# kamerkaya/SUPerman

Hardware: AMD Instinct MI355X
Metric: Gray-code subset-steps/sec (dense n=40, d=0.5) at 1/2/4/8 MI355X; rel-err vs CPU (higher is better)
Workload: dtype f64; 1 GPU; dense Ryser/Gray-code exact permanent (-p4/-p6 path), n=40 d=0.50 (double/40_0.50_0), 2^39 Gray steps per step; n=40, kernel_request=dense, preprocessing=0, jit=1, walk=segmented (pattern-specialised), parallelism=dp1: contiguous wave-chunk shards + one RCCL all-reduce

## Files before the change

### superman_amd/csrc/engine.hpp

```cpp
#pragma once
#include <stdint.h>
#include <cstdio>
#include <memory>
#include <mutex>
#include <functional>
#include <string>
#include <vector>

#include "../../include/superman.h"
#include "kernels.hpp"

namespace sup {

void set_error(const std::string& msg);
const char* last_error();
bool env_on(const char* name, bool dflt);

int to_double(const void* mat, sup_dtype t, int n, std::vector<double>& out);

void nw_start(const double* A, int n, double* x0, double* p0);

constexpr int kMaxCachedBits = 4;

enum SegCensus {
// ... 8 lines not shown
  kCenSharedCopy,
  kCenSharedForm,
  kCenHiAdd,
  kCenHiCopy,
  kCenHiForm,
  kCenStart,
  kSegCensusN
};

struct Layout {
  int L;
  int m;
  int h;
  bool fixed = false;
  int cc_cap = kMaxCachedBits;
  uint64_t chunks() const { return 1ull << h; }
};
Layout default_layout(int n);
Layout layout_with_walk(int n, int walk_log2);

struct ProdTree {
  std::vector<int> item_row;
  std::vector<uint32_t> item_sig;
  int tail_lo = 0, tail_hi = 0;
  std::vector<int> a, b;
  std::vector<uint32_t> sig;
  std::vector<uint8_t> item_live, node_live;
  int items() const { return (int)item_row.size(); }
  int K() const { return (int)a.size(); }
  int root() const { return K() ? items() + K() - 1 : (items() ? 0 : -1); }
// ... 28 lines not shown
  int seg_hi = 0;
  double seg_census[kSegCensusN] = {};
  double seg_skip = 0.0;
  int seg_regs = 0;
  int seg_budget = 0;
  std::vector<int> jofs;
  std::vector<double> jtab;
  size_t seg_cbase = 0;
  bool start_tab_on = false;
  std::vector<double> start_tab;
  int seg_kp = 4;
  std::string jit_src;
  uint64_t jit_key = 0;
  uint64_t uid = 0;
  std::vector<int> seg_order;
  bool seg_loop_scratch = false;
};

struct SegChoice {
  std::vector<int> order;
  int b = 0;
  int budget = 0;
  int cc_cap = kMaxCachedBits;
  int hi = 0;
};

int make_plan(const double* A, int n, WalkKind kind, bool identity_map, const Layout& lay, Plan& P,
              const SegChoice* choice = nullptr);

std::vector<int> greedy_walk_order(const double* A, int n, int count);
bool skip_walk_order(const double* A, int n, const Layout& lay, std::vector<int>& out,
                     const std::vector<int>* baseline, double factor);
int improve_sparse_plan(const double* A, int n, const Layout& lay, Plan& P);
int plan_threads();

std::vector<int> seg_walk_order(const double* A, int n, int m, int count, int* b_out, int cc_cap = kMaxCachedBits);
double seg_skip_estimate(const double* A, int n, const std::vector<int>& order, int m, int samples);
double seg_skip_fraction_plan(const Plan& P, int samples);
std::vector<int> seg_row_order(const double* A, int n, const std::vector<int>& walk);
int build_seg(Plan& P, int fixed_budget = 0, int fixed_hi = 0);
bool seg_choice_load(uint64_t key, int* m, SegChoice* c);
bool seg_choice_exists(uint64_t key);
double seg_cold_model(int n);
double seg_cold_predict(int n);
void seg_cost_store(int n, double seconds);
double seg_cost_ratio_load();
void seg_choice_store(uint64_t key, int m, const SegChoice& c);
int auto_decision_load(uint64_t key);
int auto_decision_store(uint64_t key, int seg);
uint64_t jit_toolchain_hash();
int seg_static_bits(int m);
double seg_cx(const Plan& P, int r, uint32_t S);
double seg_cy(const Plan& P, int r, uint32_t S);
double seg_walk_cost(const Plan& P);
int jit_occupancy(int dev, const Plan& P, int* blocks_per_cu, double* compile_ms);
// ... 313 lines not shown
```

### superman_amd/csrc/jit.cpp

```cpp
#include <dlfcn.h>
#include <hip/hiprtc.h>
#include <sched.h>
#include <spawn.h>
#include <sys/stat.h>
#include <sys/wait.h>
#include <unistd.h>

#include <cerrno>

#include <algorithm>
#include <cstring>
#include <fstream>
#include <iterator>
#include <atomic>
#include <chrono>
#include <cmath>
#include <cstdio>
#include <cstdlib>
#include <map>
#include <queue>
#include <memory>
#include <condition_variable>
#include <mutex>
#include <sstream>
// ... 84 lines not shown
  int regs = 0;
  ProdTree outer, inner;
};

inline uint64_t freq(uint32_t s, int b, int cc) {
  uint64_t v = 0;
  for (int c = cc; c <= b && c < 9; ++c)
    if ((s >> c) & 1u) v += c < b ? (1ull << (b - 1 - c)) : 1ull;
  return v;
}

constexpr int kRegs3 = 90;
static const int kRegsMax = std::getenv("SUP_JIT_REGMAX") ? std::atoi(std::getenv("SUP_JIT_REGMAX")) : 170;
constexpr double kOcc2Penalty = 1.02;

SegFit seg_fit(const SegRows& R, int cc, int budget, int budget_hi = -1, SegFit* fit_hi = nullptr) {
  SegFit f;
  f.cc = cc;
  const ClassWeights W(R.b, cc);
  std::vector<int> orow, irow;
  for (int r = R.len0; r < R.r_end; ++r) orow.push_back(r);
  for (int r = 0; r < R.s_end; ++r) irow.push_back(r);
  f.outer = make_tree(orow, R.rsig, R.r_end, R.n, W);
  f.inner = make_tree(irow, R.rsig, R.s_end, R.len0, W);
  struct Val {
    int parent = -1;
    int kids[2] = {-1, -1};
    double fr = 0;
    int cop = 1;
    double own = 0;
    int store = 0;
    bool live = true, fixed = false;
    double F = 0;
  };
// ... 52 lines not shown
      rg += cD;
    }
    *regs = rg;
    return ops;
  };
  for (auto& v : V)
    if (v.live && !v.fixed && v.parent >= 0 && V[v.parent].fr * V[v.parent].cop == v.fr * v.cop) v.live = false;
  for (const int rt : {bx + f.inner.root(), by + f.inner.root()})
    if (f.inner.root() >= 0)
      for (int k : V[rt].kids)
        if (k >= 0 && V[k].live && !V[k].fixed && fD * cD == V[k].fr * V[k].cop) V[k].live = false;
  int regs = 0;
  double ops = total(&regs);
  auto out = [&](SegFit& g, double ops_now, int regs_now) {
    g.cc = cc;
    g.outer = f.outer, g.inner = f.inner;
    auto put = [&](ProdTree& t, int base, int bit) {
      t.item_live.assign(t.items(), 0);
      t.node_live.assign(t.K(), 0);
      for (int j = 0; j < t.items(); ++j)
        if (V[base + j].live && !V[base + j].fixed) t.item_live[j] |= (uint8_t)(1u << bit);
      for (int i = 0; i < t.K(); ++i)
        if (V[base + t.items() + i].live) t.node_live[i] |= (uint8_t)(1u << bit);
    };
    put(g.outer, bo, 0);
    put(g.inner, bx, 0);
    for (int j = 0; j < g.inner.items(); ++j)
      if (V[by + j].live && !V[by + j].fixed) g.inner.item_live[j] |= 2u;
    for (int i = 0; i < g.inner.K(); ++i)
      if (V[by + g.inner.items() + i].live) g.inner.node_live[i] |= 2u;
    g.ops = (ops_now / (double)(1u << R.b) + 1.0) / 2.0;
    g.regs = regs_now;
  };
  bool took_hi = fit_hi == nullptr;
  auto nearest_live = [&](int i) {
    int a = V[i].parent;
    while (a >= 0 && !V[a].live) a = V[a].parent;
    return a;
  };
  auto delta = [&](int i) {
    const int a = nearest_live(i);
    const double fa = a >= 0 ? V[a].fr : fD, ca = a >= 0 ? V[a].cop : cD;
    return V[i].F * (fa * ca / V[i].cop - V[i].fr);
  };
  typedef std::tuple<double, int, int> Entry;
  std::priority_queue<Entry, std::vector<Entry>, std::greater<Entry>> heap;
  std::vector<int> ver(V.size(), 0);
  std::vector<double> dlt(V.size(), 0.0);
  auto push = [&](int i) {
    if (!V[i].live || V[i].fixed) return;
    dlt[i] = delta(i);
    heap.push(Entry{dlt[i] / V[i].store, i, ++ver[i]});
  };
  for (int i = 0; i < (int)V.size(); ++i) push(i);
  std::vector<int> stack;
  for (;;) {
    while (!heap.empty() && std::get<2>(heap.top()) != ver[std::get<1>(heap.top())]) heap.pop();
    const int best = heap.empty() ? -1 : std::get<1>(heap.top());
    const double bd = best < 0 ? 0.0 : dlt[best];
    if (!took_hi && (best < 0 || (bd > 1e-9 && regs <= budget_hi))) out(*fit_hi, ops, regs), took_hi = true;
    if (best < 0 || (bd > 1e-9 && regs <= budget)) break;
    heap.pop();
    V[best].live = false;
    ++ver[best];
    ops += bd, regs -= V[best].store;
    for (int p = V[best].parent; p >= 0; p = V[p].parent) {
      V[p].F += (double)V[p].cop / V[best].cop * V[best].F;
      if (V[p].live) {
        push(p);
        break;
      }
    }
    stack.assign(1, best);
    while (!stack.empty()) {
      const int u = stack.back();
      stack.pop_back();
// ... 8 lines not shown
  out(f, ops, regs);
  return f;
}

std::atomic<long> g_fit_calls{0};
int search_budget() {
  static const int b = std::getenv("SUP_JIT_SEARCH_BUDGET") ? std::atoi(std::getenv("SUP_JIT_SEARCH_BUDGET")) : kRegsMax;
  return b;
}

int max_cached() {
  const char* e = std::getenv("SUP_JIT_MAXCC");
  return e ? std::max(0, std::min(kMaxCachedBits, std::atoi(e))) : kMaxCachedBits;
}

SegFit seg_best(const SegRows& R, int cc_max, int regs_max = kRegsMax) {
  ++g_fit_calls;
  SegFit best;
  double bscore = 1e300;
  for (int cc = 0; cc <= std::min(cc_max, std::max(0, R.b - 1)); ++cc) {
    SegFit hi;
    SegFit lo = seg_fit(R, cc, kRegs3, regs_max, &hi);
    for (SegFit* f : {&lo, &hi}) {
      if (f->regs > regs_max && cc > 0) continue;
      const double score = f->ops * (f->regs <= kRegs3 ? 1.0 : kOcc2Penalty) * (f->regs > regs_max ? 2.0 : 1.0);
      if (score < bscore) bscore = score, best = std::move(*f);
    }
  }
  return best;
}

SegRows seg_rows_of(const double* A, int n, const std::vector<int>& walk, int b) {
  SegRows R;
  R.n = n, R.m = (int)walk.size();
  const std::vector<int> order = seg_row_order(A, n, walk);
  auto nz = [&](int row, int c) { return A[(size_t)row * n + c] != 0.0; };
  R.touched.assign(R.m, {});
  std::vector<char> any1(n, 0);
  for (int k = 0; k < R.m; ++k)
// ... 49 lines not shown
  std::atomic<size_t> next{0};
  auto worker = [&]() {
    for (size_t i = next++; i < count; i = next++) fn(i);
  };
  std::vector<std::thread> th;
  for (int t = 1; t < std::min({plan_threads(), (int)count, max_threads}); ++t) th.emplace_back(worker);
  worker();
  for (auto& t : th) t.join();
}

int seg_search_starts(int n) {
  if (const char* e = std::getenv("SUP_JIT_STARTS")) return std::max(1, std::atoi(e));
  return std::ldexp(1.0, n - 1) * (2.0 * n + 1.0) / 3.7e13 >= 1.0 ? 32 : 3;
}

std::vector<int> seg_walk_order(const double* A, int n, int m, int count, int* b_out, int cc_cap) {
  cc_cap = std::min(cc_cap, max_cached());
  const int nb = n - 1;
  m = std::min(m, nb);
  count = std::min(std::max(count, m), nb);
  std::vector<int> nnz(n, 0);
  for (int c = 0; c < nb; ++c)
    for (int i = 0; i < n; ++i) nnz[c] += A[(size_t)i * n + c] != 0.0;
  auto extend = [&](std::vector<int> order, int upto) {
    std::vector<char> used(n, 0), placed(n, 0);
    for (int c : order) {
      used[c] = 1;
      for (int i = 0; i < n; ++i) placed[i] |= A[(size_t)i * n + c] != 0.0;
    }
    while ((int)order.size() < upto) {
      int best = -1, bnew = 1 << 30;
      for (int c = 0; c < nb; ++c) {
        if (used[c]) continue;
        int nw = 0;
        for (int i = 0; i < n; ++i) nw += !placed[i] && A[(size_t)i * n + c] != 0.0;
        if (nw < bnew || (nw == bnew && nnz[c] < nnz[best])) best = c, bnew = nw;
      }
      used[best] = 1;
      order.push_back(best);
      for (int i = 0; i < n; ++i) placed[i] |= A[(size_t)i * n + best] != 0.0;
    }
    return order;
  };
  auto cost = [&](const std::vector<int>& o, int b) {
    if (nnz[o[0]] == 0) return 1e300;
    if (m < 3) return 0.0;
    const SegFit f = seg_best(seg_rows_of(A, n, std::vector<int>(o.begin(), o.begin() + m), b), cc_cap,
                              search_budget());
    return seg_block_bytes(f, b) > kMaxBlockBytes ? 1e300 : seg_score(f);
  };
  if (m == 0) {
    if (b_out) *b_out = 0;
    return extend({}, count);
  }
  const std::vector<int> cands = seg_b_candidates(m);
  std::vector<std::vector<int>> bests(cands.size());
  std::vector<std::vector<std::pair<double, std::vector<int>>>> finals(cands.size());
  std::vector<double> bcosts(cands.size(), 1e300);
  std::vector<std::vector<std::pair<double, std::vector<int>>>> starts(cands.size());
  auto rank_starts = [&](size_t ci) {
    const int b = cands[ci];
    for (int f = 0; f < nb; ++f) {
      std::vector<int> o = extend({f}, m);
      starts[ci].push_back({cost(o, b), std::move(o)});
    }
// ... 40 lines not shown
    std::atomic<size_t> next{0};
    auto worker = [&]() {
      for (size_t ti = next++; ti < tasks.size(); ti = next++) descend(ti);
    };
    std::vector<std::thread> th;
    for (int t = 1; t < std::min<int>(plan_threads(), (int)tasks.size()); ++t) th.emplace_back(worker);
    worker();
    for (auto& t : th) t.join();
  }
  for (size_t ci = 0; ci < cands.size(); ++ci) finals[ci].clear();
  for (size_t ti = 0; ti < tasks.size(); ++ti) {
    const size_t ci = tasks[ti].first;
    if (bests[ci].empty() || results[ti].first < bcosts[ci] - 1e-12) bcosts[ci] = results[ti].first, bests[ci] = results[ti].second;
    finals[ci].push_back(results[ti]);
  }
  size_t gi = 0;
  for (size_t ci = 1; ci < cands.size(); ++ci)
    if (bcosts[ci] < bcosts[gi] - 1e-12) gi = ci;
  bool integral = true;
  for (size_t i = 0; i < (size_t)n * n && integral; ++i) integral = A[i] == std::floor(A[i]);
  constexpr int kPolishSamples = 8192;
  constexpr int kPolishEvals = 48;
  const int need_free = std::min(3, std::max(0, nb - count));
  auto balanced = [&](const std::vector<int>& full) {
    std::vector<char> wrow(n, 0), used(n, 0);
    for (int k = 0; k < m; ++k)
      for (int i = 0; i < n; ++i) wrow[i] |= A[(size_t)i * n + full[k]] != 0.0;
    for (int c : full) used[c] = 1;
    int free_cols = 0;
    for (int c = 0; c < nb; ++c) {
      if (used[c]) continue;
      bool f = true;
      for (int i = 0; i < n && f; ++i) f = wrow[i] || A[(size_t)i * n + c] == 0.0;
// ... 26 lines not shown
      double bops = cur_ops;
      for (size_t t = 0; t < trials.size() && (int)t < kPolishEvals; ++t) {
        if (cur_ops * 0.85 * std::get<0>(trials[t]) >= best) break;
        const std::vector<int>& o = std::get<2>(trials[t]);
        if (!balanced(extend(o, count))) continue;
        const double keep = 1.0 - seg_skip_estimate(A, n, extend(o, count), m, kPolishSamples);
        const double ops = std::get<1>(trials[t]) ? cur_ops : cost(std::vector<int>(o.begin(), o.begin() + m), bb);
        if (ops < 1e300 && ops * keep < best - 1e-12) best = ops * keep, bi = (int)t, bops = ops;
      }
      if (bi < 0) break;
      beff = best, cur = std::get<2>(trials[bi]), cur_ops = bops;
    }
    bo = extend(cur, count);
    return beff;
  };
  if (integral && count >= m + std::min(6, nb - m)) {
    double beff = 1e300;
    std::vector<int> bo;
    int bb = cands[gi];
    std::vector<std::tuple<double, int, std::vector<int>>> ranked;
    for (size_t ci = 0; ci < cands.size(); ++ci)
      for (const auto& fc : finals[ci]) {
        if (fc.first >= 1e300) continue;
        const std::vector<int> full = extend(fc.second, count);
        const double eff = balanced(full) ? fc.first * (1.0 - seg_skip_estimate(A, n, full, m, kPolishSamples)) : 1e300;
        if (std::getenv("SUP_JIT_VERBOSE"))
          std::fprintf(stderr, "  candidate b=%d ops=%.4f skip=%.3f eff=%.4f\n", cands[ci], fc.first,
                       1.0 - eff / fc.first, eff);
        ranked.emplace_back(eff, cands[ci], full);
        if (eff < beff - 1e-12) beff = eff, bo = full, bb = cands[ci];
// ... 17 lines not shown
          th.emplace_back([&, i] { effs[i] = polish(std::get<2>(starts[i]), std::get<1>(starts[i]), std::get<0>(starts[i])); });
        for (auto& t : th) t.join();
        if (std::getenv("SUP_JIT_VERBOSE"))
          for (size_t i = 0; i < starts.size(); ++i) {
            const std::vector<int>& o = std::get<2>(starts[i]);
            const double ops = cost(std::vector<int>(o.begin(), o.begin() + m), std::get<1>(starts[i]));
            std::fprintf(stderr, "  polished #%zu b=%d eff=%.4f ops=%.4f eff@16384=%.4f\n", i, std::get<1>(starts[i]),
                         effs[i], ops, ops * (1.0 - seg_skip_estimate(A, n, o, m, 16384)));
          }
        size_t bi = 0;
        for (size_t i = 1; i < starts.size(); ++i)
          if (effs[i] < effs[bi] - 1e-12) bi = i;
        beff = effs[bi], bb = std::get<1>(starts[bi]), bo = std::get<2>(starts[bi]);
        if (std::getenv("SUP_JIT_VERBOSE")) std::fprintf(stderr, "  polished eff=%.4f\n", beff);
      }
      if (b_out) *b_out = bb;
      return bo;
    }
  }
  if (b_out) *b_out = cands[gi];
  return extend(bests[gi], count);
}

double seg_skip_fraction_plan(const Plan& P, int samples) {
  const int n = P.n, L = P.lay.L, m = P.lay.m, nb = n - 1;
  const int tail_lo = P.seg_start.empty() ? n : P.seg_start.back();
  if (tail_lo >= n) return 0.0;
  for (const double v : P.cols)
    if (v != std::floor(v)) return 0.0;
  const int h = nb - L - m;
  int skipped = 0;
  std::vector<double> base(n - tail_lo);
  for (int s = 0; s < samples; ++s) {
    const uint64_t a = h > 0 ? ((uint64_t)s * 0x9E3779B97F4A7C15ull) >> (64 - std::min(h, 63)) : 0;
    const uint64_t g = a ^ (a >> 1);
    for (int r = tail_lo; r < n; ++r) {
// ... 923 lines not shown
  const unsigned hb = (unsigned)(P.lay.L + P.lay.m);
  P.start_tab.assign((size_t)C * NP, 0.0);
  const size_t blocks = (size_t)std::min<uint64_t>(C, 64);
  parallel_tasks(blocks, [&](size_t b) {
    for (uint64_t ga = C * b / blocks; ga < C * (b + 1) / blocks; ++ga) {
      double* x = P.start_tab.data() + (size_t)ga * NP;
      for (int j = 0; j < NP; ++j) x[j] = P.x0[j];
      for (uint64_t h = ga ^ (ga >> 1); h; h &= h - 1) {
        const double* col = P.cols.data() + (size_t)(2u * (hb + (unsigned)__builtin_ctzll(h))) * NP;
        for (int j = 0; j < n; ++j) x[j] += col[j];
      }
    }
  });
}

int build_seg(Plan& P, int fixed_budget, int fixed_hi) {
  const int n = P.n, L = P.lay.L, m = P.lay.m;
  if (m < 3) {
    set_error("segmented walk needs >= 3 walk bits");
    return SUP_EINVAL;
  }
  if (P.cols.empty()) return SUP_EINVAL;
  P.start_tab.clear();
  P.start_tab_on = !std::getenv("SUP_JIT_NO_START_TAB") && P.lay.m <= kStartTabMaxWalkBits &&
                   (double)P.lay.chunks() * P.NP * sizeof(double) <= (double)kStartTabMaxBytes;
  P.touched.assign(m, {});
  P.seg_start.assign(1, 0);
  std::vector<char> seen(n, 0);
  int R = 0;
  for (int k = 0; k < m; ++k) {
    const double* col = P.cols.data() + (size_t)(2 * (L + k)) * P.NP;
    for (int j = 0; j < n; ++j)
// ... 45 lines not shown
    }
  }
  P.dyn_rows.clear();
  {
    std::vector<char> in(n, 0);
    for (int k = P.seg_b + 1; k < m; ++k)
      for (int r : P.touched[k]) in[r] = 1;
    for (int j = 0; j < n; ++j)
      if (in[j]) P.dyn_rows.push_back(j);
  }
  SegRows SR;
  SR.n = n, SR.m = m, SR.touched = P.touched;
  SR.len0 = P.seg_start[1], SR.s_end = P.sub_start.back(), SR.r_end = P.seg_start.back();
  seg_rows_finish(SR, P.seg_b);
  const int cc_cap = std::min(max_cached(), P.lay.cc_cap);
  auto finish = [&SR, &cc_cap, n, L, m](Plan& Q, int budget, int hi) {
    SegFit f;
    if (const char* e = std::getenv("SUP_JIT_CC"))
      f = seg_fit(SR, std::max(0, std::min({std::atoi(e), SR.b - 1, kMaxCachedBits})), budget);
    else f = seg_best(SR, cc_cap, budget);
    if (const char* e = std::getenv("SUP_JIT_STORAGE")) f = seg_fit(SR, f.cc, std::max(0, std::atoi(e)));
    Q.outer_tree = std::move(f.outer);
    Q.inner_tree = std::move(f.inner);
    Q.seg_cc = f.cc;
    Q.seg_model_ops = f.ops;
    Q.seg_regs = f.regs;
    Q.seg_budget = budget;
    Q.jofs.assign(m, 0);
    Q.jtab.clear();
    for (int k = 0; k < m; ++k) {
      const std::vector<int>& t = Q.touched[k];
      const size_t blk = (t.size() + 7) & ~(size_t)7;
      Q.jofs[k] = (int)Q.jtab.size();
      Q.jtab.resize(Q.jtab.size() + 2 * std::max<size_t>(blk, 8), 0.0);
      for (size_t i = 0; i < t.size(); ++i) {
        Q.jtab[Q.jofs[k] + i] = Q.cols[(size_t)(2 * (L + k)) * Q.NP + t[i]];
        Q.jtab[Q.jofs[k] + blk + i] = Q.cols[(size_t)(2 * (L + k) + 1) * Q.NP + t[i]];
      }
    }
    Q.seg_cbase = Q.jtab.size();
    Q.seg_kp = 4;
    if (const char* e = std::getenv("SUP_JIT_KP")) Q.seg_kp = std::max(1, std::atoi(e));
    const int hi_max = std::min(3, m - 1 - Q.seg_b);
    if (const char* e = std::getenv("SUP_JIT_HI")) hi = std::max(0, std::min(3, std::atoi(e)));
    bool neg_zero = false;
    for (int j = 0; j < n; ++j) neg_zero = neg_zero || (Q.x0[j] == 0.0 && std::signbit(Q.x0[j]));
    if (neg_zero) hi = 0;
    auto generate = [&Q](int h, std::string* src) {
      Q.seg_hi = h;
      auto g = std::make_unique<Gen>(Q);
      *src = g->source();
      return g;
    };
    auto total = [](const Gen& g) {
      double ops = 0.0;
      for (int c = 0; c < kCenStart; ++c) ops += g.census[c];
      return ops;
    };
    int taken = hi < 0 ? 0 : std::min(hi, hi_max);
// ... 29 lines not shown
    const int rc = jit_code_scan(P, &s);
    std::fprintf(stderr, "  fixed budget %d: ops %.4f rc %d vgprs %d spills %d scratch %dB (loop %d of %d insts)\n",
                 P.seg_budget, P.seg_ops, rc, s.vgprs, s.vgpr_spills, s.scratch_bytes, s.loop_scratch, s.loop_insts);
  }
  if (!fixed && walk_s < 0.01 && P.seg_cc > 3) {
    CodeScan s;
    P.seg_loop_scratch = jit_code_scan(P, &s) != SUP_OK || s.loop_scratch != 0;
  }
  auto ladder = [&](int hi, Plan& out) -> int {
    std::vector<int> budgets;
    for (int b2 = kRegs3 + 12; b2 <= kRegsMax + 60; b2 += 8) budgets.push_back(b2);
    std::vector<Plan> cand(budgets.size(), P);
    parallel_tasks(budgets.size(), [&](size_t i) { finish(cand[i], budgets[i], hi); });
    std::vector<size_t> idx;
    for (size_t i = 0; i < cand.size(); ++i) {
      bool dup = false;
      for (size_t j : idx) dup = dup || cand[j].jit_key == cand[i].jit_key;
      if (!dup) idx.push_back(i);
    }
    std::vector<CodeScan> scans(cand.size());
    std::vector<int> src(cand.size(), SUP_EHIP);
    std::vector<char> done(cand.size(), 0);
    auto compile_one = [&](size_t i) {
      if (done[i]) return;
      const auto t0 = std::chrono::steady_clock::now();
      const double own = t_compile_ms;
      src[i] = jit_code_scan(cand[i], &scans[i]);
      t_compile_ms = own + std::chrono::duration<double, std::milli>(std::chrono::steady_clock::now() - t0).count();
      done[i] = 1;
    };
    auto clean = [&](size_t i) { return done[i] && src[i] == SUP_OK && scans[i].loop_scratch == 0; };
    size_t pp = 0;
    for (size_t k = 0; k < idx.size(); ++k)
// ... 142 lines not shown
```

### superman_amd/csrc/jit_compile.cpp

```cpp
#include <dlfcn.h>
#include <hip/hip_runtime.h>
#include <hip/hiprtc.h>
#include <sched.h>
#include <signal.h>
#include <spawn.h>
#include <sys/stat.h>
#include <sys/wait.h>
#include <unistd.h>

#include <algorithm>
#include <atomic>
#include <cerrno>
#include <chrono>
#include <condition_variable>
#include <cstdio>
#include <cstdlib>
#include <cstring>
#include <fstream>
#include <map>
#include <memory>
#include <mutex>
#include <sstream>
#include <string>
#include <thread>
// ... 382 lines not shown

uint64_t jit_toolchain_hash() {
  static const uint64_t h = toolchain_hash_impl();
  return h;
}

bool seg_choice_load(uint64_t key, int* m, SegChoice* c) {
  const std::string dir = cache_dir();
  if (dir.empty()) return false;
  std::vector<char> buf;
  if (!read_file(dir + "/plan_" + key_hex(key) + ".txt", buf)) return false;
  buf.push_back('\0');
  std::istringstream in(buf.data());
  std::string tag;
  int ver = 0, cnt = 0;
  if (!(in >> tag >> ver >> *m >> c->b >> c->budget >> c->cc_cap >> c->hi >> cnt) || tag != "supseg" || ver != 4 || cnt < 1 ||
      cnt > 64 || c->hi < 0 || c->hi > 3 || c->cc_cap < 0 || c->cc_cap > kMaxCachedBits)
    return false;
  c->order.resize(cnt);
  for (int& v : c->order)
    if (!(in >> v) || v < 0 || v > 63) return false;
  return true;
}

bool seg_choice_exists(uint64_t key) {
  const std::string dir = cache_dir();
  struct stat sb;
  return !dir.empty() && ::stat((dir + "/plan_" + key_hex(key) + ".txt").c_str(), &sb) == 0;
}

void seg_choice_store(uint64_t key, int m, const SegChoice& c) {
  const std::string dir = cache_dir();
  if (dir.empty() || c.order.empty()) return;
  std::ostringstream o;
  o << "supseg 4 " << m << ' ' << c.b << ' ' << c.budget << ' ' << c.cc_cap << ' ' << c.hi << ' ' << c.order.size();
  for (int v : c.order) o << ' ' << v;
  o << '\n';
  const std::string str = o.str();
  write_file_atomic(dir, "plan_" + key_hex(key) + ".txt", std::vector<char>(str.begin(), str.end()));
}

int auto_decision_load(uint64_t key) {
  const std::string dir = cache_dir();
  if (dir.empty()) return -1;
  std::vector<char> buf;
  if (!read_file(dir + "/auto_" + key_hex(key) + ".txt", buf)) return -1;
  buf.push_back('\0');
  std::istringstream in(buf.data());
  std::string tag;
  int ver = 0, v = -1;
// ... 56 lines not shown
```

### superman_amd/csrc/plan.cpp

```cpp
#include "engine.hpp"

#include <algorithm>
#include <atomic>
#include <chrono>
#include <cmath>
#include <cstdio>
#include <cstdlib>
#include <cstring>
#include <map>
#include <memory>
#include <mutex>
#include <thread>
#include <tuple>

#include <unistd.h>

namespace sup {

static thread_local std::string g_err;
void set_error(const std::string& msg) { g_err = msg; }
const char* last_error() { return g_err.c_str(); }

bool env_on(const char* name, bool dflt) {
  const char* e = std::getenv(name);
// ... 342 lines not shown
      for (int v : o) {
        if (v < 0 || v >= nb || seen[v]) return false;
        seen[v] = 1;
      }
      return true;
    };
    if (given_order) {
      if (!valid_order(choice->order)) {
        set_error("walk column order: not m + L distinct flippable columns");
        return SUP_EINVAL;
      }
      order = choice->order;
    } else if (kind == kWalkSeg && choice && valid_order(choice->order) && choice->b >= 0 && choice->b <= m) {
      order = choice->order;
      segb = choice->b;
    } else {
      order = kind == kWalkSeg ? seg_walk_order(A, n, m, m + L, &segb, lay.cc_cap) : greedy_walk_order(A, n, m + L);
    }
    P.seg_b = segb;
    if (kind == kWalkSeg) P.seg_order.assign(order.begin(), order.begin() + (m + L));
    std::vector<char> used(n, 0);
    for (int k = 0; k < m; ++k) P.colmap[L + k] = order[k], used[order[k]] = 1;
    for (int e = 0; e < L; ++e) P.colmap[e] = order[m + e], used[order[m + e]] = 1;
    int e = L + m;
    std::vector<char> top(n, 0);
    if (kind == kWalkSeg || given_order) {
      std::vector<char> wrow(n, 0);
      for (int k = 0; k < (given_order ? m + L : m); ++k)
        for (int i = 0; i < n; ++i) wrow[i] |= A[(size_t)i * n + order[k]] != 0.0;
      for (int c = 0; c < nb && P.integral; ++c) {
        top[c] = 1;
        for (int i = 0; i < n; ++i)
          if (!wrow[i] && A[(size_t)i * n + c] != 0.0) top[c] = 0;
      }
    }
// ... 48 lines not shown

  P.umask = 0;
  for (int j = 0; j < n; ++j) {
    const int i = P.rowperm[j];
    bool lane_touched = false;
    for (int e = 0; e < L; ++e)
      if (A[(size_t)i * n + P.colmap[e]] != 0.0) lane_touched = true;
    if (!lane_touched) P.umask |= 1ull << j;
    uint64_t rm = 0;
    for (int k = 0; k < m; ++k)
      if (A[(size_t)i * n + P.colmap[L + k]] != 0.0) rm |= 1ull << k;
    P.rowmask[j] = rm;
    if ((kind == kWalkSparse || kind == kWalkDense) && !lane_touched && rm == 0 && !no_chunk_ends())
      P.chunk_ends |= 1ull << j;
  }
  if (kind == kWalkSeg) return build_seg(P, choice ? choice->budget : 0, choice ? choice->hi : 0);
  return SUP_OK;
}

static constexpr double kJitMinSavingSec = 3.0;
static constexpr double kAutoRuns = 4.0;
static constexpr double kJitWarmSavingSec = 0.1;
static constexpr int kJitWarmMinN = 30;

static int plan_for_uncached(const double* A, int n, sup_kernel kernel, const Layout& lay, Plan& P, int jit,
                             int ndev, int dev, double min_saving);
static double auto_min_saving(const double* A, int n, const Layout& lay, int jit);

static constexpr double kSegStartOps = 2048.0;

static constexpr int kSegMinChunkBits = 14;
// ... 19 lines not shown
  const int32_t head[] = {7 , n, lay.L, lay.m, (int32_t)lay.fixed, (int32_t)integral};
  f.bytes(head, sizeof head);
  if (integral) {
    f.bytes(A, nn * sizeof(double));
  } else {
    std::vector<unsigned char> pat((nn + 7) / 8, 0);
    for (size_t i = 0; i < nn; ++i)
      if (A[i] != 0.0) pat[i / 8] |= (unsigned char)(1u << (i % 8));
    f.bytes(pat.data(), pat.size());
  }
  const uint64_t k = knob_hash();
  f.bytes(&k, sizeof k);
  return f.h;
}

static int make_seg_plan(const double* A, int n, const Layout& lay, Plan& P) {
  const uint64_t dkey = seg_disk_key(A, n, lay);
  {
    int m2 = 0;
    SegChoice c;
    if (seg_choice_load(dkey, &m2, &c) && m2 >= 3 && m2 <= lay.m + lay.h && (!lay.fixed || m2 == lay.m)) {
      Layout l2 = lay;
      l2.m = m2;
      l2.h = lay.m + lay.h - m2;
      l2.cc_cap = c.cc_cap;
      if (make_plan(A, n, kWalkSeg, false, l2, P, &c) == SUP_OK) return SUP_OK;
    }
  }
  const auto t_cold = std::chrono::steady_clock::now();
  auto plan = [A, n](const Layout& l, Plan& Q) {
    int r = make_plan(A, n, kWalkSeg, false, l, Q);
    if (r == SUP_OK && Q.seg_loop_scratch && l.cc_cap > 3) {
      Layout l3 = l;
      l3.cc_cap = 3;
      r = make_plan(A, n, kWalkSeg, false, l3, Q);
    }
    return r;
  };
  int rc = plan(lay, P);
  if (rc) return rc;
  if (!lay.fixed) {
    const int mmax = std::min(lay.m + lay.h - kSegMinChunkBits, 31);
    int m2 = lay.m;
    while (m2 < mmax && std::ldexp(P.seg_model_ops, m2) < 32.0 * kSegStartOps) ++m2;
    if (m2 != lay.m) {
      Layout l2 = lay;
      l2.m = m2;
      l2.h = lay.m + lay.h - m2;
      Plan s2;
      if (plan(l2, s2) == SUP_OK) {
        auto eff = [](const Plan& q) {
          return (1.0 - q.seg_skip) * (q.seg_model_ops + std::ldexp(kSegStartOps, -q.lay.m));
        };
        if (eff(s2) < eff(P)) P = std::move(s2);
      }
    }
  }
  SegChoice c;
  c.order = P.seg_order;
  c.b = P.seg_b;
  c.budget = P.seg_budget;
  c.hi = P.seg_hi;
  c.cc_cap = P.lay.cc_cap;
  seg_choice_store(dkey, P.lay.m, c);
  const double cold_s = std::chrono::duration<double>(std::chrono::steady_clock::now() - t_cold).count();
  seg_cost_store(n, cold_s);
  if (std::getenv("SUP_JIT_VERBOSE"))
    std::fprintf(stderr, "cold segmented plan n=%d: %.3f s (compiles %.3f s wall on this thread)\n", n, cold_s,
                 jit_compile_ms_thread() * 1e-3);
  return SUP_OK;
}

namespace {
struct PlanKey {
  uint64_t hash;
  int n, kernel, L, m, jit, ndev;
  bool fixed;
  uint64_t knobs;
  bool operator<(const PlanKey& o) const {
    return std::tie(hash, n, kernel, L, m, jit, ndev, fixed, knobs) <
           std::tie(o.hash, o.n, o.kernel, o.L, o.m, o.jit, o.ndev, o.fixed, o.knobs);
// ... 92 lines not shown
    active = jit == 0 && n >= kJitWarmMinN && walk_s >= kJitWarmSavingSec;
    if (!active) return;
    key = seg_disk_key(A, n, lay) ^ (0x9e3779b97f4a7c15ull * (uint64_t)(1 + (int)kernel)) ^
          ((uint64_t)std::max(ndev, 1) << 48);
    recorded = auto_decision_load(key);
  }
  bool store(bool seg) const {
    if (active && recorded < 0) return auto_decision_store(key, seg ? 1 : 0) == 1;
    return seg;
  }
};

static int plan_for_uncached(const double* A, int n, sup_kernel kernel, const Layout& lay, Plan& P, int jit,
                             int ndev, int dev, double min_saving) {
  std::vector<WalkKind> kinds;
  auto make_seg = [&](Plan& s) { return make_seg_plan(A, n, lay, s); };
  switch (kernel) {
    case SUP_KERNEL_SKIPPER: {
      int rc = make_plan(A, n, kWalkSkip, false, lay, P);
      if (rc) return rc;
      const bool integral = P.integral;
      if (integral && n >= 10 &&
          ops_seconds(gray_steps(n), walk_cost(P), kSkipEfficiency * kLaneOpsPerSec) >= kSkipSearchMinSec) {
        SegChoice c;
        Plan Q;
        if (skip_walk_order(A, n, lay, c.order, nullptr, 0.5) && make_plan(A, n, kWalkSkip, false, lay, Q, &c) == SUP_OK)
          P = std::move(Q);
      }
      if (jit < 0 || n < 10 || lay.m < 3) return SUP_OK;
      const double steps = gray_steps(n, ndev);
      double skip_cost = walk_cost(P) / (integral ? kSkipPriceEfficiency : 1.0);
// ... 105 lines not shown
```

Measured before the change: 2966 billion gray-steps/s.

## Add deep simulated-annealing walk-order search for segmented JIT plans

Adds a deep search mode for the segmented walk order. For large n, or when JIT is requested, it runs parallel simulated-annealing walks over column orders, seeded from the plain search's finalists, and prunes weak b candidates between rounds. The deep order is compiled and checked against the plain order, and the one with the lower modeled effective ops is kept. The aim is fewer per-step operations in the generated kernel, at the cost of much longer cold planning time. It also bumps the cached choice format and adds an ops-only early exit to the fit.

```diff
diff --git a/superman_amd/csrc/engine.hpp b/superman_amd/csrc/engine.hpp
--- a/superman_amd/csrc/engine.hpp
+++ b/superman_amd/csrc/engine.hpp
@@ -46,6 +46,8 @@
   int h;
   bool fixed = false;
   int cc_cap = kMaxCachedBits;
+  bool deep = false;
+  bool order_only = false;
   uint64_t chunks() const { return 1ull << h; }
 };
 Layout default_layout(int n);
@@ -104,6 +106,9 @@
   uint64_t jit_key = 0;
   uint64_t uid = 0;
   std::vector<int> seg_order;
+  int seg_search = 0;
+  std::vector<int> seg_plain_order;
+  int seg_plain_b = 0;
   bool seg_loop_scratch = false;
 };
 
@@ -113,6 +118,8 @@
   int budget = 0;
   int cc_cap = kMaxCachedBits;
   int hi = 0;
+  int search = 0;
+  double must_beat = 1e300;
 };
 
 int make_plan(const double* A, int n, WalkKind kind, bool identity_map, const Layout& lay, Plan& P,
@@ -124,11 +131,20 @@
 int improve_sparse_plan(const double* A, int n, const Layout& lay, Plan& P);
 int plan_threads();
 
-std::vector<int> seg_walk_order(const double* A, int n, int m, int count, int* b_out, int cc_cap = kMaxCachedBits);
+struct SegSearch {
+  bool deep = false;
+  bool deep_ran = false;
+  SegChoice plain;
+  std::vector<SegChoice> per_b;
+};
+std::vector<int> seg_walk_order(const double* A, int n, int m, int count, int* b_out, int cc_cap = kMaxCachedBits,
+                                SegSearch* search = nullptr);
+bool seg_search_deep(int n, bool asked);
+int deep_budget();
 double seg_skip_estimate(const double* A, int n, const std::vector<int>& order, int m, int samples);
 double seg_skip_fraction_plan(const Plan& P, int samples);
 std::vector<int> seg_row_order(const double* A, int n, const std::vector<int>& walk);
-int build_seg(Plan& P, int fixed_budget = 0, int fixed_hi = 0);
+int build_seg(Plan& P, int fixed_budget = 0, int fixed_hi = 0, double must_beat = 1e300);
 bool seg_choice_load(uint64_t key, int* m, SegChoice* c);
 bool seg_choice_exists(uint64_t key);
 double seg_cold_model(int n);
diff --git a/superman_amd/csrc/jit.cpp b/superman_amd/csrc/jit.cpp
--- a/superman_amd/csrc/jit.cpp
+++ b/superman_amd/csrc/jit.cpp
@@ -122,10 +122,17 @@
 static const int kRegsMax = std::getenv("SUP_JIT_REGMAX") ? std::atoi(std::getenv("SUP_JIT_REGMAX")) : 170;
 constexpr double kOcc2Penalty = 1.02;
 
-SegFit seg_fit(const SegRows& R, int cc, int budget, int budget_hi = -1, SegFit* fit_hi = nullptr) {
+SegFit seg_fit(const SegRows& R, int cc, int budget, int budget_hi = -1, SegFit* fit_hi = nullptr,
+               bool ops_only = false) {
   SegFit f;
   f.cc = cc;
-  const ClassWeights W(R.b, cc);
+  static const std::vector<ClassWeights> kWeights = [] {
+    std::vector<ClassWeights> t;
+    for (int b = 0; b <= 8; ++b)
+      for (int c = 0; c <= kMaxCachedBits; ++c) t.emplace_back(b, c);
+    return t;
+  }();
+  const ClassWeights& W = kWeights[(size_t)std::min(R.b, 8) * (kMaxCachedBits + 1) + std::min(cc, kMaxCachedBits)];
   std::vector<int> orow, irow;
   for (int r = R.len0; r < R.r_end; ++r) orow.push_back(r);
   for (int r = 0; r < R.s_end; ++r) irow.push_back(r);
@@ -208,7 +215,10 @@
   double ops = total(&regs);
   auto out = [&](SegFit& g, double ops_now, int regs_now) {
     g.cc = cc;
-    g.outer = f.outer, g.inner = f.inner;
+    g.ops = (ops_now / (double)(1u << R.b) + 1.0) / 2.0;
+    g.regs = regs_now;
+    if (ops_only) return;
+    if (&g != &f) g.outer = f.outer, g.inner = f.inner;
     auto put = [&](ProdTree& t, int base, int bit) {
       t.item_live.assign(t.items(), 0);
       t.node_live.assign(t.K(), 0);
@@ -223,8 +233,6 @@
       if (V[by + j].live && !V[by + j].fixed) g.inner.item_live[j] |= 2u;
     for (int i = 0; i < g.inner.K(); ++i)
       if (V[by + g.inner.items() + i].live) g.inner.node_live[i] |= 2u;
-    g.ops = (ops_now / (double)(1u << R.b) + 1.0) / 2.0;
-    g.regs = regs_now;
   };
   bool took_hi = fit_hi == nullptr;
   auto nearest_live = [&](int i) {
@@ -254,6 +262,10 @@
     const double bd = best < 0 ? 0.0 : dlt[best];
     if (!took_hi && (best < 0 || (bd > 1e-9 && regs <= budget_hi))) out(*fit_hi, ops, regs), took_hi = true;
     if (best < 0 || (bd > 1e-9 && regs <= budget)) break;
+    if (ops_only && took_hi && fit_hi && (ops / (double)(1u << R.b) + 1.0) / 2.0 > fit_hi->ops * kOcc2Penalty) {
+      f.ops = 1e300, f.regs = regs;
+      return f;
+    }
     heap.pop();
     V[best].live = false;
     ++ver[best];
@@ -292,15 +304,16 @@
   return e ? std::max(0, std::min(kMaxCachedBits, std::atoi(e))) : kMaxCachedBits;
 }
 
-SegFit seg_best(const SegRows& R, int cc_max, int regs_max = kRegsMax) {
+SegFit seg_best(const SegRows& R, int cc_max, int regs_max = kRegsMax, int cc_min = 0, bool ops_only = false) {
   ++g_fit_calls;
   SegFit best;
   double bscore = 1e300;
-  for (int cc = 0; cc <= std::min(cc_max, std::max(0, R.b - 1)); ++cc) {
+  cc_max = std::min(cc_max, std::max(0, R.b - 1));
+  for (int cc = std::min(cc_min, cc_max); cc <= cc_max; ++cc) {
     SegFit hi;
-    SegFit lo = seg_fit(R, cc, kRegs3, regs_max, &hi);
+    SegFit lo = seg_fit(R, cc, kRegs3, regs_max, &hi, ops_only);
     for (SegFit* f : {&lo, &hi}) {
-      if (f->regs > regs_max && cc > 0) continue;
+      if (f->regs > regs_max && cc > std::min(cc_min, cc_max)) continue;
       const double score = f->ops * (f->regs <= kRegs3 ? 1.0 : kOcc2Penalty) * (f->regs > regs_max ? 2.0 : 1.0);
       if (score < bscore) bscore = score, best = std::move(*f);
     }
@@ -380,7 +393,31 @@
   return std::ldexp(1.0, n - 1) * (2.0 * n + 1.0) / 3.7e13 >= 1.0 ? 32 : 3;
 }
 
-std::vector<int> seg_walk_order(const double* A, int n, int m, int count, int* b_out, int cc_cap) {
+bool seg_search_deep(int n, bool asked) {
+  if (const char* e = std::getenv("SUP_JIT_SEARCH")) {
+    if (!std::strcmp(e, "plain")) return false;
+    if (!std::strcmp(e, "deep")) return true;
+  }
+  return asked && std::ldexp(1.0, n - 1) * (2.0 * n + 1.0) / 3.7e13 >= 1.0;
+}
+
+constexpr int kDeepBudget = 198;
+int deep_budget() {
+  if (const char* e = std::getenv("SUP_JIT_SEARCH_BUDGET")) return std::atoi(e);
+  if (const char* e = std::getenv("SUP_JIT_BUDGET")) return std::max(1, std::atoi(e));
+  return kDeepBudget;
+}
+
+static int env_int(const char* name, int dflt) {
+  const char* e = std::getenv(name);
+  return e ? std::atoi(e) : dflt;
+}
+static double env_dbl(const char* name, double dflt) {
+  const char* e = std::getenv(name);
+  return e ? std::atof(e) : dflt;
+}
+
+std::vector<int> seg_walk_order(const double* A, int n, int m, int count, int* b_out, int cc_cap, SegSearch* search) {
   cc_cap = std::min(cc_cap, max_cached());
   const int nb = n - 1;
   m = std::min(m, nb);
@@ -408,13 +445,16 @@
     }
     return order;
   };
-  auto cost = [&](const std::vector<int>& o, int b) {
+  int price = search_budget();
+  auto cost_at = [&](const std::vector<int>& o, int b, int budget, int cc_min, int cc_max, int* cc_out) {
     if (nnz[o[0]] == 0) return 1e300;
     if (m < 3) return 0.0;
-    const SegFit f = seg_best(seg_rows_of(A, n, std::vector<int>(o.begin(), o.begin() + m), b), cc_cap,
-                              search_budget());
+    const SegFit f = seg_best(seg_rows_of(A, n, std::vector<int>(o.begin(), o.begin() + m), b), cc_max, budget, cc_min,
+                              true);
+    if (cc_out) *cc_out = f.cc;
     return seg_block_bytes(f, b) > kMaxBlockBytes ? 1e300 : seg_score(f);
   };
+  auto cost = [&](const std::vector<int>& o, int b) { return cost_at(o, b, price, 0, cc_cap, nullptr); };
   if (m == 0) {
     if (b_out) *b_out = 0;
     return extend({}, count);
@@ -485,9 +525,6 @@
     if (bests[ci].empty() || results[ti].first < bcosts[ci] - 1e-12) bcosts[ci] = results[ti].first, bests[ci] = results[ti].second;
     finals[ci].push_back(results[ti]);
   }
-  size_t gi = 0;
-  for (size_t ci = 1; ci < cands.size(); ++ci)
-    if (bcosts[ci] < bcosts[gi] - 1e-12) gi = ci;
   bool integral = true;
   for (size_t i = 0; i < (size_t)n * n && integral; ++i) integral = A[i] == std::floor(A[i]);
   constexpr int kPolishSamples = 8192;
@@ -544,6 +581,10 @@
     bo = extend(cur, count);
     return beff;
   };
+  auto choose = [&](int* b_chosen) -> std::vector<int> {
+  size_t gi = 0;
+  for (size_t ci = 1; ci < cands.size(); ++ci)
+    if (bcosts[ci] < bcosts[gi] - 1e-12) gi = ci;
   if (integral && count >= m + std::min(6, nb - m)) {
     double beff = 1e300;
     std::vector<int> bo;
@@ -591,12 +632,187 @@
         beff = effs[bi], bb = std::get<1>(starts[bi]), bo = std::get<2>(starts[bi]);
         if (std::getenv("SUP_JIT_VERBOSE")) std::fprintf(stderr, "  polished eff=%.4f\n", beff);
       }
-      if (b_out) *b_out = bb;
+      *b_chosen = bb;
       return bo;
     }
   }
-  if (b_out) *b_out = cands[gi];
+  *b_chosen = cands[gi];
   return extend(bests[gi], count);
+  };
+  int b_plain = 0;
+  const bool deep = seg_search_deep(n, search && search->deep) && m >= 3;
+  if (!deep) {
+    std::vector<int> o = choose(&b_plain);
+    if (b_out) *b_out = b_plain;
+    return o;
+  }
+  const bool want_plain = search != nullptr;
+  std::vector<int> plain_order;
+  if (want_plain) plain_order = choose(&b_plain);
+  price = deep_budget();
+  const int kTasks = std::max(1, env_int("SUP_JIT_DEEP_TASKS", 16));
+  const int kEvals = std::max(0, env_int("SUP_JIT_DEEP_EVALS", 12000));
+  const int kRounds = std::max(1, env_int("SUP_JIT_DEEP_ROUNDS", 4));
+  const int kKeep = std::max(1, env_int("SUP_JIT_DEEP_KEEP", 4));
+  const double kT0 = env_dbl("SUP_JIT_DEEP_T0", 0.15), kT1 = env_dbl("SUP_JIT_DEEP_T1", 0.005);
+  const int kSeeds = std::max(1, env_int("SUP_JIT_DEEP_SEEDS", 8));
+  const double kWiden = env_dbl("SUP_JIT_DEEP_WIDEN", 3.0);
+  const double kDeepMargin = env_dbl("SUP_JIT_DEEP_MARGIN", 1.04);
+  typedef std::pair<double, std::vector<int>> Priced;
+  std::vector<std::vector<Priced>> seeds(cands.size());
+  {
+    std::vector<std::pair<size_t, Priced*>> rp;
+    std::vector<std::vector<Priced>> st1 = starts;
+    for (size_t ci = 0; ci < cands.size(); ++ci) {
+      for (auto& fc : finals[ci]) rp.push_back({ci, &fc});
+      for (auto& fc : st1[ci]) rp.push_back({ci, &fc});
+    }
+    parallel_tasks(rp.size(), [&](size_t i) { rp[i].second->first = cost(rp[i].second->second, cands[rp[i].first]); });
+    for (size_t ci = 0; ci < cands.size(); ++ci) {
+      bcosts[ci] = 1e300, bests[ci].clear();
+      for (const auto& fc : finals[ci])
+        if (bests[ci].empty() || fc.first < bcosts[ci] - 1e-12) bcosts[ci] = fc.first, bests[ci] = fc.second;
+      for (const auto* src : {&finals[ci], &st1[ci]})
+        for (const auto& fc : *src) {
+          bool dup = fc.first >= 1e300;
+          for (const auto& q : seeds[ci]) dup = dup || q.second == fc.second;
+          if (!dup) seeds[ci].push_back(fc);
+        }
+      std::stable_sort(seeds[ci].begin(), seeds[ci].end(), [](const Priced& x, const Priced& y) { return x.first < y.first; });
+      if ((int)seeds[ci].size() > kSeeds) seeds[ci].resize(kSeeds);
+      if (std::getenv("SUP_JIT_VERBOSE") && !seeds[ci].empty())
+        std::fprintf(stderr, "  deep seeds b=%d: %.4f .. %.4f at budget %d\n", cands[ci], seeds[ci][0].first,
+                     seeds[ci].back().first, price);
+    }
+  }
+  struct Walk {
+    std::vector<int> cur, best;
+    double vcur = 1e300, vbest = 1e300;
+    int ccur = 0;
+    uint64_t rs = 0;
+  };
+  std::vector<std::pair<size_t, size_t>> dtasks;
+  for (size_t ci = 0; ci < cands.size(); ++ci)
+    for (size_t t = 0; t < (size_t)kTasks; ++t)
+      if (!seeds[ci].empty()) dtasks.push_back({ci, t});
+  std::vector<Walk> walks(dtasks.size());
+  std::vector<char> live_b(cands.size(), 1);
+  const auto t_deep = std::chrono::steady_clock::now();
+  long evals_done = 0;
+  const double cool = kEvals > 1 ? std::pow(kT1 / kT0, 1.0 / (kEvals - 1)) : 1.0;
+  for (int round = 0; round < kRounds; ++round) {
+    const int e0 = (int)((long)kEvals * round / kRounds), e1 = (int)((long)kEvals * (round + 1) / kRounds);
+    parallel_tasks(dtasks.size(), [&](size_t ti) {
+      const size_t ci = dtasks[ti].first, t = dtasks[ti].second;
+      if (!live_b[ci]) return;
+      const int b = cands[ci];
+      Walk& w = walks[ti];
+      if (round == 0) {
+        w.rs = (uint64_t)(t + 1) * 0xD1342543DE82EF95ull + (uint64_t)b * 0x632BE59BD9B4E019ull;
+        const Priced& seed = seeds[ci][t % seeds[ci].size()];
+        w.cur.assign(seed.second.begin(), seed.second.begin() + m);
+        w.vcur = cost_at(w.cur, b, price, 0, cc_cap, &w.ccur);
+        w.best = w.cur, w.vbest = w.vcur;
+      }
+      auto rnd = [&w]() {
+        uint64_t z = (w.rs += 0x9E3779B97F4A7C15ull);
+        z = (z ^ (z >> 30)) * 0xBF58476D1CE4E5B9ull;
+        z = (z ^ (z >> 27)) * 0x94D049BB133111EBull;
+        return z ^ (z >> 31);
+      };
+      std::vector<int> o;
+      double T = kT0 * std::pow(cool, e0);
+      for (int e = e0; e < e1; ++e, T *= cool) {
+        int a, c;
+        o = w.cur;
+        std::vector<int>::iterator it;
+        do {
+          a = (int)(rnd() % (uint64_t)m);
+          c = (int)(rnd() % (uint64_t)(nb - 1));
+          if (c >= w.cur[a]) ++c;
+          it = std::find(o.begin(), o.end(), c);
+        } while (a > b && it != o.end() && it - o.begin() > b);
+        if (it != o.end()) std::swap(o[a], *it);
+        else o[a] = c;
+        int cc = w.ccur;
+        double v = cost_at(o, b, price, cc, cc, nullptr);
+        const double u = (double)(rnd() >> 11) * (1.0 / 9007199254740992.0);
+        if (v < 1e300 && v <= w.vcur + kWiden * T)
+          for (const int c2 : {w.ccur - 1, w.ccur + 1}) {
+            if (c2 < 0 || c2 > std::min(cc_cap, b - 1)) continue;
+            const double v2 = cost_at(o, b, price, c2, c2, nullptr);
+            if (v2 < v) v = v2, cc = c2;
+          }
+        if (v >= 1e300 || (v > w.vcur && u >= std::exp((w.vcur - v) / T))) continue;
+        w.cur = o, w.vcur = v, w.ccur = cc;
+        if (v < w.vbest - 1e-12) w.vbest = v, w.best = w.cur;
+      }
+    });
+    double round_min = 1e300;
+    for (size_t ti = 0; ti < dtasks.size(); ++ti)
+      if (live_b[dtasks[ti].first]) round_min = std::min(round_min, walks[ti].vbest), evals_done += e1 - e0;
+    if (round + 1 == kRounds) break;
+    for (size_t ci = 0; ci < cands.size(); ++ci) {
+      if (!live_b[ci]) continue;
+      std::vector<size_t> rank;
+      for (size_t ti = 0; ti < dtasks.size(); ++ti)
+        if (dtasks[ti].first == ci) rank.push_back(ti);
+      if (rank.empty()) continue;
+      std::stable_sort(rank.begin(), rank.end(), [&](size_t x, size_t y) { return walks[x].vbest < walks[y].vbest; });
+      if (walks[rank[0]].vbest > round_min * kDeepMargin) {
+        live_b[ci] = 0;
+        continue;
+      }
+      std::vector<size_t> keep;
+      for (size_t ti : rank) {
+        bool dup = false;
+        for (size_t q : keep) dup = dup || walks[q].best == walks[ti].best;
+        if (!dup) keep.push_back(ti);
+        if ((int)keep.size() == kKeep) break;
+      }
+      std::vector<Walk> from;
+      for (size_t q : keep) from.push_back(walks[q]);
+      size_t k = 0;
+      for (size_t ti = 0; ti < dtasks.size(); ++ti)
+        if (dtasks[ti].first == ci) {
+          const Walk& f = from[k++ % from.size()];
+          walks[ti].cur = walks[ti].best = f.best, walks[ti].vcur = walks[ti].vbest = f.vbest;
+        }
+    }
+  }
+  std::vector<Priced> dres(dtasks.size());
+  parallel_tasks(dtasks.size(), [&](size_t ti) {
+    dres[ti] = {walks[ti].best.empty() ? 1e300 : cost(walks[ti].best, cands[dtasks[ti].first]), walks[ti].best};
+  });
+  if (std::getenv("SUP_JIT_VERBOSE")) {
+    const double s = std::chrono::duration<double>(std::chrono::steady_clock::now() - t_deep).count();
+    std::fprintf(stderr, "  deep search: %ld evaluations at budget %d in %.2f s (%.0f evaluations/s)\n", evals_done, price, s,
+                 (double)evals_done / std::max(s, 1e-9));
+  }
+  for (size_t ti = 0; ti < dtasks.size(); ++ti) {
+    const size_t ci = dtasks[ti].first;
+    if (dres[ti].second.empty()) continue;
+    if (dres[ti].first < bcosts[ci] - 1e-12) bcosts[ci] = dres[ti].first, bests[ci] = dres[ti].second;
+    finals[ci].push_back(dres[ti]);
+    if (std::getenv("SUP_JIT_VERBOSE"))
+      std::fprintf(stderr, "  deep b=%d task %zu: %.4f\n", cands[ci], dtasks[ti].second, dres[ti].first);
+  }
+  int b_deep = 0;
+  std::vector<int> deep_order = choose(&b_deep);
+  if (search) {
+    search->deep_ran = true;
+    search->plain.order = plain_order, search->plain.b = b_plain;
+    search->per_b.clear();
+    if (!integral)
+      for (size_t ci = 0; ci < cands.size(); ++ci)
+        if (!bests[ci].empty() && bcosts[ci] < 1e300) {
+          SegChoice c;
+          c.order = extend(bests[ci], count), c.b = cands[ci], c.search = 1;
+          search->per_b.push_back(std::move(c));
+        }
+  }
+  if (b_out) *b_out = b_deep;
+  return deep_order;
 }
 
 double seg_skip_fraction_plan(const Plan& P, int samples) {
@@ -1550,8 +1766,10 @@
   });
 }
 
-int build_seg(Plan& P, int fixed_budget, int fixed_hi) {
+int build_seg(Plan& P, int fixed_budget, int fixed_hi, double must_beat) {
   const int n = P.n, L = P.lay.L, m = P.lay.m;
+  const bool ranking = fixed_hi < 0;
+  if (fixed_hi == -2) fixed_hi = 0;
   if (m < 3) {
     set_error("segmented walk needs >= 3 walk bits");
     return SUP_EINVAL;
@@ -1627,7 +1845,7 @@
   SR.len0 = P.seg_start[1], SR.s_end = P.sub_start.back(), SR.r_end = P.seg_start.back();
   seg_rows_finish(SR, P.seg_b);
   const int cc_cap = std::min(max_cached(), P.lay.cc_cap);
-  auto finish = [&SR, &cc_cap, n, L, m](Plan& Q, int budget, int hi) {
+  auto finish = [&SR, &cc_cap, n, L, m, ranking](Plan& Q, int budget, int hi) {
     SegFit f;
     if (const char* e = std::getenv("SUP_JIT_CC"))
       f = seg_fit(SR, std::max(0, std::min({std::atoi(e), SR.b - 1, kMaxCachedBits})), budget);
@@ -1655,7 +1873,7 @@
     Q.seg_kp = 4;
     if (const char* e = std::getenv("SUP_JIT_KP")) Q.seg_kp = std::max(1, std::atoi(e));
     const int hi_max = std::min(3, m - 1 - Q.seg_b);
-    if (const char* e = std::getenv("SUP_JIT_HI")) hi = std::max(0, std::min(3, std::atoi(e)));
+    if (const char* e = ranking ? nullptr : std::getenv("SUP_JIT_HI")) hi = std::max(0, std::min(3, std::atoi(e)));
     bool neg_zero = false;
     for (int j = 0; j < n; ++j) neg_zero = neg_zero || (Q.x0[j] == 0.0 && std::signbit(Q.x0[j]));
     if (neg_zero) hi = 0;
@@ -1715,9 +1933,13 @@
     parallel_tasks(budgets.size(), [&](size_t i) { finish(cand[i], budgets[i], hi); });
     std::vector<size_t> idx;
     for (size_t i = 0; i < cand.size(); ++i) {
-      bool dup = false;
+      bool dup = cand[i].seg_ops >= must_beat;
       for (size_t j : idx) dup = dup || cand[j].jit_key == cand[i].jit_key;
       if (!dup) idx.push_back(i);
+    }
+    if (idx.empty()) {
+      set_error("segmented walk: no budget of this order has fewer ops than the kernel it is set against");
+      return (int)SUP_EHIP;
     }
     std::vector<CodeScan> scans(cand.size());
     std::vector<int> src(cand.size(), SUP_EHIP);
diff --git a/superman_amd/csrc/jit_compile.cpp b/superman_amd/csrc/jit_compile.cpp
--- a/superman_amd/csrc/jit_compile.cpp
+++ b/superman_amd/csrc/jit_compile.cpp
@@ -420,8 +420,9 @@
   std::istringstream in(buf.data());
   std::string tag;
   int ver = 0, cnt = 0;
-  if (!(in >> tag >> ver >> *m >> c->b >> c->budget >> c->cc_cap >> c->hi >> cnt) || tag != "supseg" || ver != 4 || cnt < 1 ||
-      cnt > 64 || c->hi < 0 || c->hi > 3 || c->cc_cap < 0 || c->cc_cap > kMaxCachedBits)
+  if (!(in >> tag >> ver) || tag != "supseg" || ver != 5) return false;
+  if (!(in >> *m >> c->b >> c->budget >> c->cc_cap >> c->hi >> c->search >> cnt) || cnt < 1 || cnt > 64 || c->hi < 0 ||
+      c->hi > 3 || c->cc_cap < 0 || c->cc_cap > kMaxCachedBits || c->search < 0 || c->search > 1)
     return false;
   c->order.resize(cnt);
   for (int& v : c->order)
@@ -439,7 +440,8 @@
   const std::string dir = cache_dir();
   if (dir.empty() || c.order.empty()) return;
   std::ostringstream o;
-  o << "supseg 4 " << m << ' ' << c.b << ' ' << c.budget << ' ' << c.cc_cap << ' ' << c.hi << ' ' << c.order.size();
+  o << "supseg 5 " << m << ' ' << c.b << ' ' << c.budget << ' ' << c.cc_cap << ' ' << c.hi << ' ' << c.search << ' '
+    << c.order.size();
   for (int v : c.order) o << ' ' << v;
   o << '\n';
   const std::string str = o.str();
diff --git a/superman_amd/csrc/plan.cpp b/superman_amd/csrc/plan.cpp
--- a/superman_amd/csrc/plan.cpp
+++ b/superman_amd/csrc/plan.cpp
@@ -7,6 +7,7 @@
 #include <cstdio>
 #include <cstdlib>
 #include <cstring>
+#include <functional>
 #include <map>
 #include <memory>
 #include <mutex>
@@ -380,11 +381,35 @@
     } else if (kind == kWalkSeg && choice && valid_order(choice->order) && choice->b >= 0 && choice->b <= m) {
       order = choice->order;
       segb = choice->b;
+      P.seg_search = choice->search;
+    } else if (kind == kWalkSeg) {
+      SegSearch search;
+      search.deep = lay.deep;
+      order = seg_walk_order(A, n, m, m + L, &segb, lay.cc_cap, &search);
+      if (search.deep_ran) {
+        P.seg_search = 1;
+        P.seg_plain_order = search.plain.order, P.seg_plain_b = search.plain.b;
+        double best = 1e300;
+        for (SegChoice& c : search.per_b) {
+          c.budget = deep_budget();
+          c.hi = std::getenv("SUP_JIT_BUDGET") ? -2 : -1;
+          c.cc_cap = lay.cc_cap;
+          Plan T;
+          Layout lt = lay;
+          lt.order_only = false;
+          if (make_plan(A, n, kind, false, lt, T, &c) != SUP_OK) continue;
+          if (std::getenv("SUP_JIT_VERBOSE"))
+            std::fprintf(stderr, "  deep candidate b=%d: census total %.4f (hi %d) at budget %d\n", c.b, T.seg_ops,
+                         T.seg_hi, c.budget);
+          if (T.seg_ops < best - 1e-12) best = T.seg_ops, order = c.order, segb = c.b;
+        }
+      }
     } else {
-      order = kind == kWalkSeg ? seg_walk_order(A, n, m, m + L, &segb, lay.cc_cap) : greedy_walk_order(A, n, m + L);
+      order = greedy_walk_order(A, n, m + L);
     }
     P.seg_b = segb;
     if (kind == kWalkSeg) P.seg_order.assign(order.begin(), order.begin() + (m + L));
+    if (kind == kWalkSeg && lay.order_only) return SUP_OK;
     std::vector<char> used(n, 0);
     for (int k = 0; k < m; ++k) P.colmap[L + k] = order[k], used[order[k]] = 1;
     for (int e = 0; e < L; ++e) P.colmap[e] = order[m + e], used[order[m + e]] = 1;
@@ -463,7 +488,8 @@
     if ((kind == kWalkSparse || kind == kWalkDense) && !lane_touched && rm == 0 && !no_chunk_ends())
       P.chunk_ends |= 1ull << j;
   }
-  if (kind == kWalkSeg) return build_seg(P, choice ? choice->budget : 0, choice ? choice->hi : 0);
+  if (kind == kWalkSeg)
+    return build_seg(P, choice ? choice->budget : 0, choice ? choice->hi : 0, choice ? choice->must_beat : 1e300);
   return SUP_OK;
 }
 
@@ -513,12 +539,16 @@
   return f.h;
 }
 
-static int make_seg_plan(const double* A, int n, const Layout& lay, Plan& P) {
+static int make_seg_plan(const double* A, int n, const Layout& lay_in, Plan& P, bool deep) {
+  Layout lay = lay_in;
+  lay.deep = deep;
+  const bool want_deep = seg_search_deep(n, deep);
   const uint64_t dkey = seg_disk_key(A, n, lay);
   {
     int m2 = 0;
     SegChoice c;
-    if (seg_choice_load(dkey, &m2, &c) && m2 >= 3 && m2 <= lay.m + lay.h && (!lay.fixed || m2 == lay.m)) {
+    if (seg_choice_load(dkey, &m2, &c) && (c.search == 1 || !want_deep) && m2 >= 3 && m2 <= lay.m + lay.h &&
+        (!lay.fixed || m2 == lay.m)) {
       Layout l2 = lay;
       l2.m = m2;
       l2.h = lay.m + lay.h - m2;
@@ -527,13 +557,44 @@
     }
   }
   const auto t_cold = std::chrono::steady_clock::now();
-  auto plan = [A, n](const Layout& l, Plan& Q) {
-    int r = make_plan(A, n, kWalkSeg, false, l, Q);
+  auto plan1 = [A, n](const Layout& l, Plan& Q, const SegChoice* c) {
+    int r = make_plan(A, n, kWalkSeg, false, l, Q, c);
     if (r == SUP_OK && Q.seg_loop_scratch && l.cc_cap > 3) {
       Layout l3 = l;
       l3.cc_cap = 3;
-      r = make_plan(A, n, kWalkSeg, false, l3, Q);
-    }
+      r = make_plan(A, n, kWalkSeg, false, l3, Q, c);
+    }
+    return r;
+  };
+  std::function<int(const Layout&, Plan&)> plan = [&](const Layout& l, Plan& Q) -> int {
+    if (!seg_search_deep(n, l.deep)) return plan1(l, Q, nullptr);
+    Layout lo = l;
+    lo.order_only = true;
+    Plan S;
+    int r = make_plan(A, n, kWalkSeg, false, lo, S);
+    if (r != SUP_OK) return r;
+    if (S.seg_search != 1) return plan1(l, Q, nullptr);
+    auto eff = [](const Plan& q) { return q.seg_ops * (1.0 - q.seg_skip); };
+    auto again_cc3 = [&](const Plan& q, int rq) { return rq == SUP_OK && q.seg_loop_scratch && l.cc_cap > 3; };
+    Layout l3 = l;
+    l3.cc_cap = 3;
+    SegChoice cp, cd;
+    cp.order = S.seg_plain_order, cp.b = S.seg_plain_b;
+    cd.order = S.seg_order, cd.b = S.seg_b;
+    cp.cc_cap = cd.cc_cap = l.cc_cap, cp.search = cd.search = 1;
+    r = make_plan(A, n, kWalkSeg, false, l, Q, &cp);
+    if (again_cc3(Q, r)) return plan(l3, Q);
+    if (cp.order == cd.order && cp.b == cd.b) return r;
+    if (r == SUP_OK && !Q.integral) cd.must_beat = Q.seg_ops;
+    Plan D;
+    const int rd = make_plan(A, n, kWalkSeg, false, l, D, &cd);
+    if (again_cc3(D, rd)) return plan(l3, Q);
+    const bool take = rd == SUP_OK && (r != SUP_OK || eff(D) < eff(Q));
+    if (std::getenv("SUP_JIT_VERBOSE"))
+      std::fprintf(stderr, "  walk-order guard: the %s search's order wins after the compiler check (plain %s %.4f, deep %s %.4f)\n",
+                   take ? "deep" : "plain", r == SUP_OK ? "ok" : "failed", r == SUP_OK ? eff(Q) : 0.0,
+                   rd == SUP_OK ? "ok" : "no kernel", rd == SUP_OK ? eff(D) : 0.0);
+    if (take) Q = std::move(D), r = SUP_OK;
     return r;
   };
   int rc = plan(lay, P);
@@ -561,9 +622,10 @@
   c.budget = P.seg_budget;
   c.hi = P.seg_hi;
   c.cc_cap = P.lay.cc_cap;
+  c.search = P.seg_search;
   seg_choice_store(dkey, P.lay.m, c);
   const double cold_s = std::chrono::duration<double>(std::chrono::steady_clock::now() - t_cold).count();
-  seg_cost_store(n, cold_s);
+  if (!P.seg_search) seg_cost_store(n, cold_s);
   if (std::getenv("SUP_JIT_VERBOSE"))
     std::fprintf(stderr, "cold segmented plan n=%d: %.3f s (compiles %.3f s wall on this thread)\n", n, cold_s,
                  jit_compile_ms_thread() * 1e-3);
@@ -686,7 +748,7 @@
 static int plan_for_uncached(const double* A, int n, sup_kernel kernel, const Layout& lay, Plan& P, int jit,
                              int ndev, int dev, double min_saving) {
   std::vector<WalkKind> kinds;
-  auto make_seg = [&](Plan& s) { return make_seg_plan(A, n, lay, s); };
+  auto make_seg = [&](Plan& s) { return make_seg_plan(A, n, lay, s, jit >= 1); };
   switch (kernel) {
     case SUP_KERNEL_SKIPPER: {
       int rc = make_plan(A, n, kWalkSkip, false, lay, P);
```

New measurement: 2962 billion gray-steps/s. About the same (-0.2%).
